# samiazirar/mvtracker

Hardware: AMD Instinct MI355X
Metric: query-points*frames/sec, 4-view 24-frame 512x512 @1024 queries (higher is better)
Workload: dtype bf16; 1 GPU; c3: 4-view synthetic 24-frame 512x512, 1024 queries, bf16 (configs[2], the metric's config); 4-view 24-frame 512x512, 1024 queries per GPU, corr K=16 x 4 levels, iters=4, 3 windows, random-init weights (seeded recipe); queries_total=1024, parallelism=query-shard x1, frame_store=bf16 rows

## Files before the change

mvtracker_amd/csrc/encoder_forward.hip:

```cpp
#include "common.h"
#include <stdlib.h>

namespace {

inline long long align256(long long b) { return (b + 255) & ~255LL; }

struct Plan {
  long long stem, z0, y, s[4], d, cat, c2, part, st, total;
  long long st_ch;
};

inline Plan plan(long long n, int H, int W, int C) {
  const long long h2 = H / 2, w2 = W / 2, hs = H / 4, ws = W / 4;
  Plan P{};
  long long o = 0;
  auto take = [&](long long bytes) { const long long at = o; o += align256(bytes); return at; };
  const long long big = n * h2 * w2 * 64 * 2;
  P.stem = take(big);
  P.z0 = take(big);
  P.y = take(big);
  const int couts[4] = {64, 96, 128, 128};
  long long hh = h2, ww = w2;
  for (int l = 0; l < 4; ++l) {
    if (l) {
      hh = (hh - 1) / 2 + 1;
      ww = (ww - 1) / 2 + 1;
    }
    P.s[l] = take(n * hh * ww * couts[l] * 2);
  }
  P.d = take(n * hs * ws * 96 * 2);
  P.cat = take(n * hs * ws * 416 * 2);
  P.c2 = take(n * hs * ws * 2 * C * 2);
  const long long slots_max = ((h2 + 7) / 8) * ((w2 + 31) / 32);
  P.st_ch = 2 * C > 256 ? 2 * C : 256;
  P.part = take(n * slots_max * P.st_ch * 2 * 4);
  P.st = take(8 * n * P.st_ch * 2 * 4);
  P.total = o;
  return P;
}

}

extern "C" long long mvt_encoder_workspace_bytes(int n, int H, int W, int C) {
  if (n <= 0 || H < 16 || W < 16 || C <= 0) return -1;
  return plan(n, H, W, C).total;
}

#define ENC_TRY(call)              \
  do {                             \
    const int rc_ = (call);        \
    if (rc_ != MVT_OK) return rc_; \
  } while (0)

int mvt_detail_conv_rows_slots(int Ho, int Wo, int tile_rows);
int mvt_detail_conv_rows_tile_rows(int ksize, int stride, int Ho);
int mvt_detail_stem7x7_rows_src(const float* in, const void* rgb, int rgb_u8, int rgb_V, int rgb_T, long long rgb_img0, const unsigned short* w,
                                int ldw, const float* bias, void* out, int n, int H, int W, int Cout, int ldo, int io_flags, float* out_partial,
                                hipStream_t stream);

static int encoder_run(const mvt_encoder_weights* w, const float* x4, const void* rgb, int rgb_u8, int rgb_V, int rgb_T, long long img0,
                       int n, int H, int W, void* out_rows, int ldo, int out_bf16, void* workspace, long long workspace_bytes, void* stream) {
  MVT_REQUIRE(w && (x4 || rgb) && out_rows && workspace && n > 0 && H >= 16 && W >= 16 && H % 4 == 0 && W % 4 == 0);
  const int C = w->latent_dim;
  MVT_REQUIRE(C > 0 && C % 32 == 0 && ldo >= C && (out_bf16 == 0 || out_bf16 == 1));
  const Plan P = plan(n, H, W, C);
  MVT_REQUIRE(workspace_bytes >= P.total && ((uintptr_t)workspace % 256) == 0);
  for (int i = 0; i < MVT_ENCODER_CONVS; ++i) MVT_REQUIRE(w->conv[i].w && w->conv[i].b);
  char* base = (char*)workspace;
  float* part = (float*)(base + P.part);
  float* stb = (float*)(base + P.st);
  const long long st_stride = (long long)n * P.st_ch * 2;
  int st_next = 0;
  auto new_st = [&]() { float* s = stb + (st_next % 8) * st_stride; ++st_next; return s; };
  const int BF = MVT_IO_IN_BF16 | MVT_IO_OUT_BF16;

  auto conv = [&](int ci, const void* in, int io_in, void* out, int hh, int ww, int cin, int cout, int k, int stride, int pad, int ld_out,
                  const float* in_stats, float** st_out, int io_out) -> int {
    const mvt_conv_weights& cw = w->conv[ci];
    const int ho = (hh + 2 * pad - k) / stride + 1, wo = (ww + 2 * pad - k) / stride + 1;
    float* pp = nullptr;
    int slots = 0;
    if (st_out) {
      slots = mvt_conv2d_stat_slots(hh, ww, cin, k, k, stride, pad, 0);
      MVT_REQUIRE(slots > 0);
      pp = part;
    }
    ENC_TRY(mvt_conv2d_bf16(in, cw.w, nullptr, cw.b, out, n, hh, ww, cin, cout, k, k, stride, pad, ld_out, MVT_ACT_NONE,
                            io_in | io_out | (w->short_workgroups ? MVT_IO_SHORT_WG : 0), in_stats, pp, stream));
    if (st_out) {
      *st_out = new_st();
      ENC_TRY(mvt_instnorm_finish_slots(pp, slots, *st_out, n, (long long)ho * wo, cout, stream));
    }
    return MVT_OK;
  };

  const int h2 = H / 2, w2 = W / 2;
  float* st_stem = nullptr;
  if (x4) {
    ENC_TRY(conv(0, x4, 0, base + P.stem, H, W, 4, 64, 7, 2, 3, 64, nullptr, &st_stem, MVT_IO_OUT_BF16));
  } else {
    const mvt_conv_weights& cw = w->conv[0];
    const int slots = mvt_detail_conv_rows_slots(h2, w2, mvt_detail_conv_rows_tile_rows(7, 2, h2));
    ENC_TRY(mvt_detail_stem7x7_rows_src(nullptr, rgb, rgb_u8, rgb_V, rgb_T, img0, cw.w, (7 * 32 + 63) & ~63, cw.b, base + P.stem, n, H, W, 64, 64,
                                        MVT_IO_OUT_BF16, part, mvt_stream(stream)));
    st_stem = new_st();
    ENC_TRY(mvt_instnorm_finish_slots(part, slots, st_stem, n, (long long)h2 * w2, 64, stream));
  }

  auto res_block = [&](int c1, int c2, int cd, const void* xin, const float* x_stats, int hh, int ww, int cin, int cout, int stride,
                       void* zout) -> int {
    const int ho = (hh + 2 - 3) / stride + 1, wo = (ww + 2 - 3) / stride + 1;
    float *s1 = nullptr, *s2 = nullptr, *sd = nullptr;
    static const bool no_fold = getenv("MVT_FOLD_DOWNSAMPLE") && atoi(getenv("MVT_FOLD_DOWNSAMPLE")) == 0;
    const bool fold = cd >= 0 && stride == 2 && !x_stats && cout % 32 == 0 && !no_fold;
    if (fold) {
      const int slots = mvt_conv2d_stat_slots(hh, ww, cin, 3, 3, 2, 1, 0);
      MVT_REQUIRE(slots > 0);
      float* part_d = part + (long long)n * slots * cout * 2;
      ENC_TRY(mvt_conv3x3s2_down_bf16(xin, w->conv[c1].w, w->conv[c1].b, w->conv[cd].w, w->conv[cd].b, base + P.y, base + P.d, n, hh, ww, cin,
                                      cout, cout, part, part_d, stream));
      s1 = new_st();
      ENC_TRY(mvt_instnorm_finish_slots(part, slots, s1, n, (long long)ho * wo, cout, stream));
      sd = new_st();
      ENC_TRY(mvt_instnorm_finish_slots(part_d, slots, sd, n, (long long)ho * wo, cout, stream));
    } else {
      ENC_TRY(conv(c1, xin, MVT_IO_IN_BF16, base + P.y, hh, ww, cin, cout, 3, stride, 1, cout, x_stats, &s1, MVT_IO_OUT_BF16));
    }
    ENC_TRY(conv(c2, base + P.y, MVT_IO_IN_BF16, zout, ho, wo, cout, cout, 3, 1, 1, cout, s1, &s2, MVT_IO_OUT_BF16));
    const void* skip = xin;
    const float* skip_stats = x_stats;
    int flags = BF | (x_stats ? MVT_APPLY_SKIP_RELU : 0);
    if (cd >= 0) {
      if (!fold) ENC_TRY(conv(cd, xin, MVT_IO_IN_BF16, base + P.d, hh, ww, cin, cout, 1, stride, 0, cout, nullptr, &sd, MVT_IO_OUT_BF16));
      skip = base + P.d;
      skip_stats = sd;
      flags = BF;
    }
    return mvt_instnorm_apply(zout, s2, skip, skip_stats, zout, n, (long long)ho * wo, cout, flags, stream);
  };

  const void* stage[4];
  int sh[4], sw[4], sc[4];
  const void* xin = base + P.stem;
  const float* xst = st_stem;
  int hh = h2, ww = w2, cin = 64;
  const int couts[4] = {64, 96, 128, 128}, strides[4] = {1, 2, 2, 2};
  for (int l = 0; l < 4; ++l) {
    const int b0 = 1 + 5 * l, cout = couts[l], stride = strides[l];
    ENC_TRY(res_block(b0, b0 + 1, l == 0 ? -1 : b0 + 2, xin, xst, hh, ww, cin, cout, stride, base + P.z0));
    hh = (hh + 2 - 3) / stride + 1;
    ww = (ww + 2 - 3) / stride + 1;
    ENC_TRY(res_block(b0 + 3, b0 + 4, -1, base + P.z0, nullptr, hh, ww, cout, cout, 1, base + P.s[l]));
    stage[l] = base + P.s[l]; sh[l] = hh; sw[l] = ww; sc[l] = cout;
    xin = base + P.s[l]; xst = nullptr; cin = cout;
  }
  const int hs = H / 4, ws = W / 4;
  ENC_TRY(mvt_concat_resize_bilinear_ac(4, stage, sh, sw, sc, base + P.cat, n, hs, ws, 416, BF, stream));
  float* st_c2 = nullptr;
  ENC_TRY(conv(21, base + P.cat, MVT_IO_IN_BF16, base + P.c2, hs, ws, 416, 2 * C, 3, 1, 1, 2 * C, nullptr, &st_c2, MVT_IO_OUT_BF16));
  ENC_TRY(conv(22, base + P.c2, MVT_IO_IN_BF16, out_rows, hs, ws, 2 * C, C, 1, 1, 0, ldo, st_c2, nullptr, out_bf16 ? MVT_IO_OUT_BF16 : 0));
  return MVT_OK;
}

extern "C" int mvt_encoder_forward(const mvt_encoder_weights* w, const float* x4, int n, int H, int W, void* out_rows, int ldo,
                                   int out_bf16, void* workspace, long long workspace_bytes, void* stream) {
  MVT_REQUIRE(x4);
  return encoder_run(w, x4, nullptr, 0, 0, 0, 0, n, H, W, out_rows, ldo, out_bf16, workspace, workspace_bytes, stream);
}

extern "C" int mvt_encoder_forward_rgb(const mvt_encoder_weights* w, const void* rgbs, int is_u8, int V, int T, long long img0, int n, int H,
                                       int W, void* out_rows, int ldo, int out_bf16, void* workspace, long long workspace_bytes,
                                       void* stream) {
  MVT_REQUIRE(rgbs && (is_u8 == 0 || is_u8 == 1) && V > 0 && T > 0 && img0 >= 0 && n > 0 && img0 + n <= (long long)V * T);
  return encoder_run(w, nullptr, rgbs, is_u8, V, T, img0, n, H, W, out_rows, ldo, out_bf16, workspace, workspace_bytes, stream);
}
```

Measured before the change: 1.010 million query-points*frames/s.

## Process encoder stem and first layer in image groups sized to cache budget

Splits the stem and layer-0 residual blocks into groups of images, sized so the three large half-resolution bf16 buffers fit an 80MB budget when short_workgroups is set; otherwise the group is the whole batch. Each group runs stem, conv, instnorm and apply back to back so the intermediates can stay resident in the last-level cache rather than spilling to HBM. Later layers still run on the full batch. In exchange it launches more, smaller kernels with less parallelism per launch, and the stats-buffer indexing gets more complex.

```diff
diff --git a/mvtracker_amd/csrc/encoder_forward.hip b/mvtracker_amd/csrc/encoder_forward.hip
--- a/mvtracker_amd/csrc/encoder_forward.hip
+++ b/mvtracker_amd/csrc/encoder_forward.hip
@@ -39,6 +39,19 @@
   return P;
 }
 
+constexpr long long GROUP_BUDGET_SHARED = 80LL << 20;
+inline int group_size(int n, int h2, int w2, int shared, int* g_out) {
+  long long g = shared ? GROUP_BUDGET_SHARED / (3LL * h2 * w2 * 64 * 2) : n;
+  if (g < 1) g = n;
+  if (const char* e = getenv("MVT_ENC_GROUP")) {
+    const long v = strtol(e, nullptr, 10);
+    if (v < 0) return MVT_ERR_ARG;
+    if (v > 0) g = v;
+  }
+  *g_out = (int)(g > n ? n : g);
+  return MVT_OK;
+}
+
 }
 
 extern "C" long long mvt_encoder_workspace_bytes(int n, int H, int W, int C) {
@@ -73,86 +86,106 @@
   int st_next = 0;
   auto new_st = [&]() { float* s = stb + (st_next % 8) * st_stride; ++st_next; return s; };
   const int BF = MVT_IO_IN_BF16 | MVT_IO_OUT_BF16;
+  const int h2 = H / 2, w2 = W / 2;
+  int g = n;
+  ENC_TRY(group_size(n, h2, w2, w->short_workgroups, &g));
+
+  int ga = 0, gn = n;
+  auto img = [&](const void* p, long long bytes_per_image) { return (char*)p + ga * bytes_per_image; };
+  auto rows_of = [&](const float* table, int ch) { return table ? table + (long long)ga * ch * 2 : nullptr; };
 
   auto conv = [&](int ci, const void* in, int io_in, void* out, int hh, int ww, int cin, int cout, int k, int stride, int pad, int ld_out,
                   const float* in_stats, float** st_out, int io_out) -> int {
     const mvt_conv_weights& cw = w->conv[ci];
     const int ho = (hh + 2 * pad - k) / stride + 1, wo = (ww + 2 * pad - k) / stride + 1;
+    const long long in_img = (long long)hh * ww * cin * (io_in & MVT_IO_IN_BF16 ? 2 : 4);
+    const long long out_img = (long long)ho * wo * ld_out * (io_out & MVT_IO_OUT_BF16 ? 2 : 4);
     float* pp = nullptr;
     int slots = 0;
     if (st_out) {
       slots = mvt_conv2d_stat_slots(hh, ww, cin, k, k, stride, pad, 0);
       MVT_REQUIRE(slots > 0);
-      pp = part;
-    }
-    ENC_TRY(mvt_conv2d_bf16(in, cw.w, nullptr, cw.b, out, n, hh, ww, cin, cout, k, k, stride, pad, ld_out, MVT_ACT_NONE,
-                            io_in | io_out | (w->short_workgroups ? MVT_IO_SHORT_WG : 0), in_stats, pp, stream));
+      pp = part + (long long)ga * slots * cout * 2;
+    }
+    ENC_TRY(mvt_conv2d_bf16(img(in, in_img), cw.w, nullptr, cw.b, img(out, out_img), gn, hh, ww, cin, cout, k, k, stride, pad, ld_out,
+                            MVT_ACT_NONE, io_in | io_out | (w->short_workgroups ? MVT_IO_SHORT_WG : 0), rows_of(in_stats, cin), pp, stream));
     if (st_out) {
       *st_out = new_st();
-      ENC_TRY(mvt_instnorm_finish_slots(pp, slots, *st_out, n, (long long)ho * wo, cout, stream));
+      ENC_TRY(mvt_instnorm_finish_slots(pp, slots, (float*)rows_of(*st_out, cout), gn, (long long)ho * wo, cout, stream));
     }
     return MVT_OK;
   };
 
-  const int h2 = H / 2, w2 = W / 2;
-  float* st_stem = nullptr;
-  if (x4) {
-    ENC_TRY(conv(0, x4, 0, base + P.stem, H, W, 4, 64, 7, 2, 3, 64, nullptr, &st_stem, MVT_IO_OUT_BF16));
-  } else {
+  auto stem = [&](float** st_stem) -> int {
+    if (x4) return conv(0, x4, 0, base + P.stem, H, W, 4, 64, 7, 2, 3, 64, nullptr, st_stem, MVT_IO_OUT_BF16);
     const mvt_conv_weights& cw = w->conv[0];
     const int slots = mvt_detail_conv_rows_slots(h2, w2, mvt_detail_conv_rows_tile_rows(7, 2, h2));
-    ENC_TRY(mvt_detail_stem7x7_rows_src(nullptr, rgb, rgb_u8, rgb_V, rgb_T, img0, cw.w, (7 * 32 + 63) & ~63, cw.b, base + P.stem, n, H, W, 64, 64,
-                                        MVT_IO_OUT_BF16, part, mvt_stream(stream)));
-    st_stem = new_st();
-    ENC_TRY(mvt_instnorm_finish_slots(part, slots, st_stem, n, (long long)h2 * w2, 64, stream));
-  }
+    float* pp = part + (long long)ga * slots * 64 * 2;
+    ENC_TRY(mvt_detail_stem7x7_rows_src(nullptr, rgb, rgb_u8, rgb_V, rgb_T, img0 + ga, cw.w, (7 * 32 + 63) & ~63, cw.b,
+                                        img(base + P.stem, (long long)h2 * w2 * 64 * 2), gn, H, W, 64, 64, MVT_IO_OUT_BF16, pp, mvt_stream(stream)));
+    *st_stem = new_st();
+    return mvt_instnorm_finish_slots(pp, slots, (float*)rows_of(*st_stem, 64), gn, (long long)h2 * w2, 64, stream);
+  };
 
   auto res_block = [&](int c1, int c2, int cd, const void* xin, const float* x_stats, int hh, int ww, int cin, int cout, int stride,
                        void* zout) -> int {
     const int ho = (hh + 2 - 3) / stride + 1, wo = (ww + 2 - 3) / stride + 1;
+    const long long in_img = (long long)hh * ww * cin * 2, out_img = (long long)ho * wo * cout * 2;
     float *s1 = nullptr, *s2 = nullptr, *sd = nullptr;
     static const bool no_fold = getenv("MVT_FOLD_DOWNSAMPLE") && atoi(getenv("MVT_FOLD_DOWNSAMPLE")) == 0;
     const bool fold = cd >= 0 && stride == 2 && !x_stats && cout % 32 == 0 && !no_fold;
     if (fold) {
       const int slots = mvt_conv2d_stat_slots(hh, ww, cin, 3, 3, 2, 1, 0);
       MVT_REQUIRE(slots > 0);
-      float* part_d = part + (long long)n * slots * cout * 2;
-      ENC_TRY(mvt_conv3x3s2_down_bf16(xin, w->conv[c1].w, w->conv[c1].b, w->conv[cd].w, w->conv[cd].b, base + P.y, base + P.d, n, hh, ww, cin,
-                                      cout, cout, part, part_d, stream));
+      float* part_3 = part + (long long)ga * slots * cout * 2;
+      float* part_d = part_3 + (long long)n * slots * cout * 2;
+      ENC_TRY(mvt_conv3x3s2_down_bf16(img(xin, in_img), w->conv[c1].w, w->conv[c1].b, w->conv[cd].w, w->conv[cd].b, img(base + P.y, out_img),
+                                      img(base + P.d, out_img), gn, hh, ww, cin, cout, cout, part_3, part_d, stream));
       s1 = new_st();
-      ENC_TRY(mvt_instnorm_finish_slots(part, slots, s1, n, (long long)ho * wo, cout, stream));
+      ENC_TRY(mvt_instnorm_finish_slots(part_3, slots, (float*)rows_of(s1, cout), gn, (long long)ho * wo, cout, stream));
       sd = new_st();
-      ENC_TRY(mvt_instnorm_finish_slots(part_d, slots, sd, n, (long long)ho * wo, cout, stream));
+      ENC_TRY(mvt_instnorm_finish_slots(part_d, slots, (float*)rows_of(sd, cout), gn, (long long)ho * wo, cout, stream));
     } else {
       ENC_TRY(conv(c1, xin, MVT_IO_IN_BF16, base + P.y, hh, ww, cin, cout, 3, stride, 1, cout, x_stats, &s1, MVT_IO_OUT_BF16));
     }
     ENC_TRY(conv(c2, base + P.y, MVT_IO_IN_BF16, zout, ho, wo, cout, cout, 3, 1, 1, cout, s1, &s2, MVT_IO_OUT_BF16));
     const void* skip = xin;
+    long long skip_img = in_img;
     const float* skip_stats = x_stats;
     int flags = BF | (x_stats ? MVT_APPLY_SKIP_RELU : 0);
     if (cd >= 0) {
       if (!fold) ENC_TRY(conv(cd, xin, MVT_IO_IN_BF16, base + P.d, hh, ww, cin, cout, 1, stride, 0, cout, nullptr, &sd, MVT_IO_OUT_BF16));
       skip = base + P.d;
+      skip_img = out_img;
       skip_stats = sd;
       flags = BF;
     }
-    return mvt_instnorm_apply(zout, s2, skip, skip_stats, zout, n, (long long)ho * wo, cout, flags, stream);
-  };
-
-  const void* stage[4];
-  int sh[4], sw[4], sc[4];
-  const void* xin = base + P.stem;
-  const float* xst = st_stem;
-  int hh = h2, ww = w2, cin = 64;
+    return mvt_instnorm_apply(img(zout, out_img), rows_of(s2, cout), img(skip, skip_img), rows_of(skip_stats, cout), img(zout, out_img), gn,
+                              (long long)ho * wo, cout, flags, stream);
+  };
+
   const int couts[4] = {64, 96, 128, 128}, strides[4] = {1, 2, 2, 2};
-  for (int l = 0; l < 4; ++l) {
+  auto layer = [&](int l, const void* xin, const float* xst, int hh, int ww, int cin) -> int {
     const int b0 = 1 + 5 * l, cout = couts[l], stride = strides[l];
     ENC_TRY(res_block(b0, b0 + 1, l == 0 ? -1 : b0 + 2, xin, xst, hh, ww, cin, cout, stride, base + P.z0));
     hh = (hh + 2 - 3) / stride + 1;
     ww = (ww + 2 - 3) / stride + 1;
-    ENC_TRY(res_block(b0 + 3, b0 + 4, -1, base + P.z0, nullptr, hh, ww, cout, cout, 1, base + P.s[l]));
-    stage[l] = base + P.s[l]; sh[l] = hh; sw[l] = ww; sc[l] = cout;
-    xin = base + P.s[l]; xst = nullptr; cin = cout;
+    return res_block(b0 + 3, b0 + 4, -1, base + P.z0, nullptr, hh, ww, cout, cout, 1, base + P.s[l]);
+  };
+
+  for (ga = 0; ga < n; ga += g) {
+    gn = n - ga < g ? n - ga : g;
+    st_next = 0;
+    float* st_stem = nullptr;
+    ENC_TRY(stem(&st_stem));
+    ENC_TRY(layer(0, base + P.stem, st_stem, h2, w2, 64));
+  }
+  ga = 0, gn = n;
+  const void* stage[4] = {base + P.s[0]};
+  int sh[4] = {h2}, sw[4] = {w2}, sc[4] = {64};
+  for (int l = 1; l < 4; ++l) {
+    ENC_TRY(layer(l, base + P.s[l - 1], nullptr, sh[l - 1], sw[l - 1], sc[l - 1]));
+    stage[l] = base + P.s[l]; sh[l] = (sh[l - 1] - 1) / 2 + 1; sw[l] = (sw[l - 1] - 1) / 2 + 1; sc[l] = couts[l];
   }
   const int hs = H / 4, ws = W / 4;
   ENC_TRY(mvt_concat_resize_bilinear_ac(4, stage, sh, sw, sc, base + P.cat, n, hs, ws, 416, BF, stream));
```

After: 1.051 million query-points*frames/s (median of 6 runs). 1.04x the previous value.
